# Restream/reindexer

Hardware: AMD Instinct MI355X
Metric: knn_queries_per_sec (higher is better)
Workload: dtype f32; 1 GPU; brute-force KNN, 10000000 x 768 fp32 per GPU, metric=ip, k=10, batch=1 (BASELINE configs[1]); rows_per_gpu=10000000, total_rows=10000000, dim=768, k=10, batch=1, rccl_ranks=0, arch=gfx950:sramecc+:xnack-

## Files before the change

include/rxgpu.h:

```cpp
#ifndef RXGPU_H
#define RXGPU_H

#include <stddef.h>
#include <stdint.h>

#ifdef __cplusplus
extern "C" {
#endif

#define RXGPU_ABI_VERSION 2

typedef enum rxgpu_status {
	RXGPU_OK = 0,
	RXGPU_ERR_PARAMS = -3,
	RXGPU_ERR_LOGIC = -4,
	RXGPU_ERR_NOMEM = -5,
	RXGPU_ERR_DEVICE = -6,
	RXGPU_ERR_NOTFOUND = -7,
	RXGPU_ERR_OVERFLOW = -8
} rxgpu_status;

typedef enum rxgpu_metric { RXGPU_METRIC_L2 = 0, RXGPU_METRIC_IP = 1, RXGPU_METRIC_COSINE = 2 } rxgpu_metric;

typedef struct rxgpu_index rxgpu_index;
// ... 31 lines not shown
uint64_t rxgpu_index_capacity(const rxgpu_index* h);
uint32_t rxgpu_index_dim(const rxgpu_index* h);
uint32_t rxgpu_index_row_stride(const rxgpu_index* h);
int rxgpu_index_metric(const rxgpu_index* h);
int rxgpu_index_device(const rxgpu_index* h);
uint64_t rxgpu_index_device_bytes(const rxgpu_index* h);


int rxgpu_search_knn(rxgpu_index* h, const float* queries, uint32_t nq, uint32_t kk, float* out_dist, uint32_t* out_row,
					 uint32_t* out_count);

int rxgpu_index_upload_row_ids(rxgpu_index* h, uint64_t first_row, uint64_t n, const int32_t* row_ids);
const void* rxgpu_index_row_ids_device(const rxgpu_index* h);
int rxgpu_search_knn_resident(rxgpu_index* h, const float* query, uint32_t kk, void** d_dist, void** d_row, void** d_count, void** stream,
							  uint32_t* entries);
uint32_t rxgpu_index_resident_contexts(rxgpu_index* h);
int rxgpu_search_knn_device(rxgpu_index* h, const void* d_queries, uint32_t nq, uint32_t kk, void* d_out_dist, void* d_out_row,
							void* d_out_count, void* stream);
int rxgpu_scan_policy(uint64_t rows, uint32_t dim, uint32_t nq, int shadow_available, int stats_finite);
int rxgpu_scan_tier(uint64_t rows, uint32_t dim, uint32_t nq, int shadow_available, int stats_finite);
int rxgpu_scan_i6(uint64_t rows, uint32_t dim, uint32_t nq, int i6_available, int stats_finite);
int rxgpu_index_last_candidates(const rxgpu_index* h, uint32_t* out_count, uint32_t* out_cap);
int rxgpu_index_inspect(rxgpu_index* h, const char* what, void* out, uint64_t cap_bytes, uint64_t* out_bytes);

int rxgpu_search_knn_subset(rxgpu_index* h, const float* queries, uint32_t nq, uint32_t kk, const uint32_t* row_ids, uint64_t n_ids,
							float* out_dist, uint32_t* out_row, uint32_t* out_count);
int rxgpu_search_knn_bitmap(rxgpu_index* h, const float* queries, uint32_t nq, uint32_t kk, const uint32_t* allowed_words,
							uint64_t n_words, float* out_dist, uint32_t* out_row, uint32_t* out_count, uint64_t* out_allowed);
int rxgpu_scan_tier_subset(uint64_t n_ids, uint32_t dim, uint32_t nq, uint32_t kk, int shadow_available, int stats_finite);

int rxgpu_index_set_lists(rxgpu_index* h, uint32_t nlist, const uint64_t* list_off, const uint32_t* list_rows);
int rxgpu_search_knn_lists(rxgpu_index* h, rxgpu_index* coarse, const float* query, uint32_t nprobe, uint32_t kk, float* out_dist,
						   uint32_t* out_row, uint32_t* out_count, uint64_t* out_scanned);
int rxgpu_search_range_lists(rxgpu_index* h, rxgpu_index* coarse, const float* query, uint32_t nprobe, float radius, int inclusive, float* out_dist,
							 uint32_t* out_row, uint64_t cap, uint64_t* out_total, uint64_t* out_scanned);

int rxgpu_ivf_assign(rxgpu_index* h, rxgpu_index* coarse, const uint32_t* row_ids, uint64_t first_row, uint64_t n, uint32_t* out_list);
int rxgpu_ivf_kmeans_step(rxgpu_index* h, rxgpu_index* coarse, const uint32_t* row_ids, uint64_t n, float* out_centroids, float* out_hassign,
						  uint32_t* out_assign);
int rxgpu_ivf_read_train_stats(rxgpu_index* h, uint64_t* rows_assigned, uint64_t* steps, double* kernel_ms, double* sums_ms);

int rxgpu_search_knn_subset_device(rxgpu_index* h, const void* d_queries, uint32_t nq, uint32_t kk, const void* d_row_ids,
								   uint64_t n_ids, void* d_out_dist, void* d_out_row, void* d_out_count, void* stream);
int rxgpu_check_row_list_device(rxgpu_index* h, const void* d_row_ids, uint64_t n_ids, void* stream, int32_t* out_ok);

int rxgpu_search_range_subset(rxgpu_index* h, const float* query, float radius, int inclusive, const uint32_t* row_ids, uint64_t n_ids,
// ... 174 lines not shown
```

reindexer_amd/capi.py:

```python
from __future__ import annotations

import ctypes as C
import os
from pathlib import Path

import numpy as np

PKG = Path(__file__).resolve().parent
LIB_PATH = PKG / "librxgpu.so"

METRIC_L2, METRIC_IP, METRIC_COSINE = 0, 1, 2
METRICS = {"l2": METRIC_L2, "ip": METRIC_IP, "inner_product": METRIC_IP, "cosine": METRIC_COSINE}

RXGPU_OK = 0
RXGPU_ERR_PARAMS = -3
RXGPU_ERR_LOGIC = -4
RXGPU_ERR_NOMEM = -5
RXGPU_ERR_DEVICE = -6
RXGPU_ERR_NOTFOUND = -7
RXGPU_ERR_OVERFLOW = -8

_vp, _u32, _u64, _i, _f = C.c_void_p, C.c_uint32, C.c_uint64, C.c_int, C.c_float
_SIGNATURES = {
    "rxgpu_last_error": (C.c_char_p, []),
# ... 17 lines not shown
    "rxgpu_index_adopt_device_rows": (_i, [_vp, _vp, _u64, _u32, _vp]),
    "rxgpu_index_move_row": (_i, [_vp, _u64, _u64]),
    "rxgpu_index_truncate": (_i, [_vp, _u64]),
    "rxgpu_index_count": (_u64, [_vp]),
    "rxgpu_index_capacity": (_u64, [_vp]),
    "rxgpu_index_dim": (_u32, [_vp]),
    "rxgpu_index_row_stride": (_u32, [_vp]),
    "rxgpu_index_metric": (_i, [_vp]),
    "rxgpu_index_device": (_i, [_vp]),
    "rxgpu_index_device_bytes": (_u64, [_vp]),
    "rxgpu_search_knn": (_i, [_vp, _vp, _u32, _u32, _vp, _vp, _vp]),
    "rxgpu_index_upload_row_ids": (_i, [_vp, _u64, _u64, _vp]),
    "rxgpu_index_row_ids_device": (_vp, [_vp]),
    "rxgpu_search_knn_resident": (_i, [_vp, _vp, _u32, C.POINTER(_vp), C.POINTER(_vp), C.POINTER(_vp), C.POINTER(_vp), C.POINTER(_u32)]),
    "rxgpu_index_resident_contexts": (_u32, [_vp]),
    "rxgpu_search_knn_device": (_i, [_vp, _vp, _u32, _u32, _vp, _vp, _vp, _vp]),
    "rxgpu_scan_policy": (_i, [_u64, _u32, _u32, _i, _i]),
    "rxgpu_scan_tier": (_i, [_u64, _u32, _u32, _i, _i]),
    "rxgpu_scan_i6": (_i, [_u64, _u32, _u32, _i, _i]),
    "rxgpu_scan_tier_subset": (_i, [_u64, _u32, _u32, _u32, _i, _i]),
    "rxgpu_scan_tier_range": (_i, [_u64, _u32, _i, _i, _i]),
    "rxgpu_index_last_candidates": (_i, [_vp, C.POINTER(_u32), C.POINTER(_u32)]),
    "rxgpu_index_inspect": (_i, [_vp, C.c_char_p, _vp, _u64, C.POINTER(_u64)]),
    "rxgpu_search_knn_subset": (_i, [_vp, _vp, _u32, _u32, _vp, _u64, _vp, _vp, _vp]),
    "rxgpu_search_knn_bitmap": (_i, [_vp, _vp, _u32, _u32, _vp, _u64, _vp, _vp, _vp, C.POINTER(_u64)]),
    "rxgpu_index_set_lists": (_i, [_vp, _u32, _vp, _vp]),
    "rxgpu_search_knn_lists": (_i, [_vp, _vp, _vp, _u32, _u32, _vp, _vp, _vp, C.POINTER(_u64)]),
    "rxgpu_search_range_lists": (_i, [_vp, _vp, _vp, _u32, C.c_float, _i, _vp, _vp, _u64, C.POINTER(_u64), C.POINTER(_u64)]),
    "rxgpu_ivf_assign": (_i, [_vp, _vp, _vp, _u64, _u64, _vp]),
    "rxgpu_ivf_kmeans_step": (_i, [_vp, _vp, _vp, _u64, _vp, _vp, _vp]),
    "rxgpu_ivf_read_train_stats": (_i, [_vp, C.POINTER(_u64), C.POINTER(_u64), C.POINTER(C.c_double), C.POINTER(C.c_double)]),
    "rxgpu_search_knn_subset_device": (_i, [_vp, _vp, _u32, _u32, _vp, _u64, _vp, _vp, _vp, _vp]),
    "rxgpu_check_row_list_device": (_i, [_vp, _vp, _u64, _vp, C.POINTER(C.c_int32)]),
    "rxgpu_search_range_subset": (_i, [_vp, _vp, _f, _i, _vp, _u64, _vp, _vp, _u64, C.POINTER(_u64)]),
    "rxgpu_merge_shards_device": (_i, [_vp, _u32, _u32, _u32, _u32, _vp, _vp, _vp, _vp]),
    "rxgpu_search_range": (_i, [_vp, _vp, _f, _i, _vp, _vp, _u64, C.POINTER(_u64)]),
    "rxgpu_distances": (_i, [_vp, _vp, _vp, _u32, _vp]),
    "rxgpu_hnsw_attach_graph": (_i, [_vp, _vp, _vp, _vp, _u64, _vp, _u32, _u32, C.c_int32, _u32, _u64]),
    "rxgpu_hnsw_update_deleted": (_i, [_vp, _vp, _u64]),
    "rxgpu_hnsw_patch_graph": (_i, [_vp, _u32, _vp, _vp, _vp, _vp, _vp, C.c_int32, _u32, _u64]),
    "rxgpu_hnsw_search_knn": (_i, [_vp, _vp, _u32, _u32, _u32, _vp, _vp, _vp]),
    "rxgpu_hnsw_search_knn_posted": (_i, [_vp, _vp, _u32, _u32, _vp, _vp, _vp, C.POINTER(C.c_int32)]),
    "rxgpu_hnsw_server_stats": (_i, [_vp, C.POINTER(_u64), C.POINTER(_u64)]),
    "rxgpu_hnsw_server_times": (_i, [_vp, C.POINTER(_u64), C.POINTER(_u64)]),
    "rxgpu_hnsw_read_stats4": (_i, [_vp, _vp]),
    "rxgpu_hnsw_attach_sq8": (_i, [_vp, _vp, _vp, _u64, _f]),
# ... 104 lines not shown
    if n < 0:
        _check(n)
    return n


def device_arch(device: int = 0) -> str:
    buf = C.create_string_buffer(256)
    _check(lib().rxgpu_device_arch(device, buf, 256))
    return buf.value.decode()


def scan_policy(rows: int, dim: int, nq: int = 1, shadow_available: bool = True, stats_finite: bool = True) -> bool:
    return bool(lib().rxgpu_scan_policy(rows, dim, nq, int(shadow_available), int(stats_finite)))


def scan_tier(rows: int, dim: int, nq: int = 1, shadow_available: bool = True, stats_finite: bool = True) -> int:
    return int(lib().rxgpu_scan_tier(rows, dim, nq, int(shadow_available), int(stats_finite)))


def scan_i6(rows: int, dim: int, nq: int = 1, i6_available: bool = True, stats_finite: bool = True) -> bool:
    return bool(lib().rxgpu_scan_i6(rows, dim, nq, int(i6_available), int(stats_finite)))


def scan_tier_range(rows: int, dim: int, listed: bool = False, shadow_available: bool = True, stats_finite: bool = True) -> int:
    return int(lib().rxgpu_scan_tier_range(rows, dim, int(listed), int(shadow_available), int(stats_finite)))


def scan_tier_subset(n_ids: int, dim: int, nq: int = 1, kk: int = 10, shadow_available: bool = True, stats_finite: bool = True) -> int:
    return int(lib().rxgpu_scan_tier_subset(n_ids, dim, nq, kk, int(shadow_available), int(stats_finite)))


def _f32c(a) -> np.ndarray:
    return np.ascontiguousarray(a, dtype=np.float32)


class VectorIndex:

    def __init__(self, metric: int | str, dim: int, capacity: int = 0, device: int = 0):
        if isinstance(metric, str):
            metric = METRICS[metric.lower()]
        self.metric, self.dim = int(metric), int(dim)
        h = _vp()
        _check(lib().rxgpu_index_create(self.metric, self.dim, capacity, device, C.byref(h)))
        self._h = h
        self._keepalive = None

# ... 483 lines not shown
```

reindexer_amd/csrc/knn_batched.hip:

```cpp
#include "knn_i8_quant.h"
#include "knn_kernels.hip.h"
#include "rxgpu_internal.h"

namespace rxgpu {

typedef float f32x16 __attribute__((ext_vector_type(16)));

constexpr int kGemmThreads = 256;
constexpr int kGemmRows = 128;
constexpr int kGemmKS = 32;
constexpr int kLdsStride = kGemmKS + 1;

template <int kMetric, int MT, int kMode, int QS>
__global__ __launch_bounds__(kGemmThreads * QS) void knn_gemm(GemmParams p) {
	extern __shared__ __attribute__((aligned(16))) float lds[];
	constexpr int kThreads = kGemmThreads * QS;
	constexpr int QB = MT / 32 / QS;
	constexpr int kQTile = MT * kLdsStride;
	constexpr int kXTile = kGemmRows * kLdsStride;
	float* q_s = lds;
	float* x_s = lds + 2 * kQTile;
	float* thr_s = x_s + 2 * kXTile;
	float* aux_s = thr_s + MT;
	constexpr int kQLoads = MT * (kGemmKS / 4) / kThreads;
// ... 230 lines not shown
	}
	for (int off = 32; off; off >>= 1) s += __shfl_xor(s, off);
	if (lane == 0) {
		const float mg = query_margin<kMetric, true>(s, dim, stats);
		q_sq[qi] = s;
		margin[qi] = mg;
		cand_cnt[qi] = (s < __builtin_inff() && mg < __builtin_inff()) ? 0u : cap + 1u;
	}
}

template <int kMetric>
__global__ __launch_bounds__(64) void knn_query_prep_i8(const float* src, uint32_t dim, float* qpad, int8_t* planes, uint32_t ld8, const unsigned int* stats,
															 float* q_sq, float* margin, float2* qinfo, uint32_t* cand_cnt, uint32_t cap,
															 const unsigned int* estats, const unsigned int* bad_flag) {
	const uint32_t qi = blockIdx.x;
	const int lane = threadIdx.x;
	const float* q = src + size_t(qi) * dim;
	float* o = qpad + size_t(qi) * ld8;
	int8_t* ph = planes + size_t(qi) * 2 * ld8;
	int8_t* pl = ph + ld8;
	float s = 0.f, mx = 0.f;
	double s64 = 0.0;
	bool bad = false;
	for (uint32_t i = lane; i < ld8; i += 64) {
		const float v = i < dim ? q[i] : 0.f;
		o[i] = v;
		if (i < dim) {
			s = __builtin_fmaf(v, v, s);
			s64 += double(v) * double(v);
			mx = fmaxf(mx, fabsf(v));
			bad |= !(fabsf(v) < __builtin_inff());
		}
	}
	for (int off = 32; off; off >>= 1) {
		s += __shfl_xor(s, off);
		s64 += __shfl_xor(s64, off);
		mx = fmaxf(mx, __shfl_xor(mx, off));
	}
	const float sq = i8_scale(mx, kI8QueryMax);
	double r64 = 0.0;
	for (uint32_t i = lane; i < ld8; i += 64) {
		const float v = i < dim ? q[i] : 0.f;
		const int t = i8_quantize(v, sq, kI8QueryMax);
		int hh, ll;
		i8_split(t, hh, ll);
		ph[i] = int8_t(hh);
		pl[i] = int8_t(ll);
		const double r = i8_residual(v, sq, t);
		r64 += r * r;
	}
	for (int off = 32; off; off >>= 1) r64 += __shfl_xor(r64, off);
	bad = __ballot(bad) != 0;
	if (lane == 0) {
		const float qn = i8_norm_up(s64), rq = i8_norm_up(r64);
		const float mg = i8_margin<kMetric>(s, dim, qn, rq, __uint_as_float(stats[0]), __uint_as_float(stats[1]), __uint_as_float(estats[0]), __uint_as_float(estats[1]));
		q_sq[qi] = s;
		qinfo[qi] = make_float2(sq, qn);
		const bool ok = !bad && stats[2] == 0 && !(bad_flag && *bad_flag != 0) && s < __builtin_inff() && qn < __builtin_inff() && mg < __builtin_inff();
		margin[qi] = ok ? mg : __builtin_inff();
		cand_cnt[qi] = ok ? 0u : cap + 1u;
	}
}

__global__ __launch_bounds__(256) void knn_sample_threshold(const float* dense, uint64_t ns, uint32_t nq, uint32_t kk, const float* margin,
															 float* thr) {
	__shared__ float s_d[4][kMaxFusedK];
	__shared__ uint32_t s_i[4][kMaxFusedK];
	const int lane = threadIdx.x & 63, wave = threadIdx.x >> 6;
	const uint32_t qi = blockIdx.x;
	WaveTopK top;
	top.init(kk);
	if (qi < nq) {
// ... 161 lines not shown
```

reindexer_amd/csrc/knn_scan.hip:

```cpp
#include <algorithm>
#include <type_traits>

#include "knn_kernels.hip.h"
#include "knn_scan_common.hip.h"
#include "rxgpu_internal.h"

#include <cstdlib>

namespace rxgpu {

typedef unsigned int u32x4 __attribute__((ext_vector_type(4)));

constexpr int kMergeThreads = 512;
constexpr int kMergeWaves = kMergeThreads / kWave;
constexpr int kMergeAhead = 8;

__device__ __forceinline__ void block_merge_and_store(WaveTopK2& top, const ScanParams& p, int lane, int wave) {
	__shared__ float s_d[kScanWaves][kMaxFusedK2];
	__shared__ uint32_t s_i[kScanWaves][kMaxFusedK2];
	s_d[wave][lane] = top.d0;
	s_i[wave][lane] = top.i0;
	s_d[wave][64 + lane] = top.d1;
	s_i[wave][64 + lane] = top.i1;
	__syncthreads();
// ... 576 lines not shown
	uint32_t b = __float_as_uint(d);
	if (b == 0x80000000u) b = 0;
	b ^= (b >> 31) ? 0xFFFFFFFFu : 0x80000000u;
	return (static_cast<unsigned long long>(b) << 32) | row;
}
__device__ __forceinline__ void merge_bitonic(unsigned long long* key, float* val, uint32_t n) {
	for (uint32_t k = 2; k <= n; k <<= 1) {
		for (uint32_t j = k >> 1; j > 0; j >>= 1) {
			for (uint32_t t = threadIdx.x; t < n / 2; t += kMergeThreads) {
				const uint32_t i = ((t & ~(j - 1)) << 1) | (t & (j - 1)), l = i | j;
				const unsigned long long x = key[i], y = key[l];
				if ((x > y) == ((i & k) == 0)) {
					key[i] = y;
					key[l] = x;
					const float vx = val[i];
					val[i] = val[l];
					val[l] = vx;
				}
			}
			__syncthreads();
		}
	}
}
template <typename TK>
__device__ void merge_by_insertion(const float* part_dist, const uint32_t* part_row, size_t base, uint32_t total, uint32_t kk, float* out_dist,
								   uint32_t* out_row, uint32_t* out_count, float* s_d, uint32_t* s_i);

template <typename TK>
__device__ __forceinline__ void merge_lists(const float* part_dist, const uint32_t* part_row, uint32_t nlists, uint32_t kk, float* out_dist, uint32_t* out_row,
											uint32_t* out_count, unsigned long long* s_key, float* s_val, uint32_t* s_np) {
	uint32_t& s_n = *s_np;
	const uint32_t tid = threadIdx.x, total = nlists * kk;
	const size_t base = size_t(blockIdx.x) * total;
	bool serial = nlists < kk || nlists > kMergeHeadsMax;
	if (!serial) {
		uint32_t n1 = 64;
		while (n1 < nlists) n1 <<= 1;
		for (uint32_t l = tid; l < n1; l += kMergeThreads) {
			unsigned long long k = ~0ull;
			if (l < nlists) {
				const uint32_t r = part_row[base + size_t(l) * kk];
				if (r != kInvalidRow) k = merge_pair_key(part_dist[base + size_t(l) * kk], r);
			}
			s_key[l] = k;
			s_val[l] = 0.f;
		}
		if (tid == 0) s_n = 0;
		__syncthreads();
		merge_bitonic(s_key, s_val, n1);
		const unsigned long long bound = s_key[kk - 1];
		__syncthreads();
		for (uint32_t l = tid; l < nlists; l += kMergeThreads) {
			const size_t at = base + size_t(l) * kk;
			for (uint32_t e = 0; e < kk; ++e) {
				const uint32_t r = part_row[at + e];
				if (r == kInvalidRow) break;
				const float d = part_dist[at + e];
				const unsigned long long k = merge_pair_key(d, r);
				if (k > bound) break;
				const uint32_t pos = atomicAdd(&s_n, 1u);
				if (pos < kMergeCandMax) {
					s_key[pos] = k;
					s_val[pos] = d;
				}
			}
		}
		__syncthreads();
		const uint32_t n = s_n;
		serial = n > kMergeCandMax;
		if (!serial) {
			uint32_t n2 = 64;
			while (n2 < n) n2 <<= 1;
			for (uint32_t q = n + tid; q < n2; q += kMergeThreads) {
				s_key[q] = ~0ull;
				s_val[q] = 0.f;
			}
			__syncthreads();
			merge_bitonic(s_key, s_val, n2);
			const uint32_t cnt = n < kk ? n : kk;
			for (uint32_t q = tid; q < kk; q += kMergeThreads) {
				out_dist[size_t(blockIdx.x) * kk + q] = q < cnt ? s_val[q] : __builtin_inff();
				out_row[size_t(blockIdx.x) * kk + q] = q < cnt ? uint32_t(s_key[q]) : kInvalidRow;
			}
			if (tid == 0 && out_count) out_count[blockIdx.x] = cnt;
			return;
		}
		__syncthreads();
	}
	merge_by_insertion<TK>(part_dist, part_row, base, total, kk, out_dist, out_row, out_count, s_val, reinterpret_cast<uint32_t*>(s_key));
}

template <typename TK>
__global__ __launch_bounds__(kMergeThreads) void knn_merge_lists(const float* part_dist, const uint32_t* part_row, uint32_t nlists, uint32_t kk,
																  float* out_dist, uint32_t* out_row, uint32_t* out_count, const uint32_t* gate_cnt,
																  uint32_t gate_cap) {
	__shared__ unsigned long long s_key[kMergeHeadsMax];
	__shared__ float s_val[kMergeHeadsMax];
	__shared__ uint32_t s_n;
	if (gate_cnt && gate_cnt[blockIdx.x] <= gate_cap) return;
	merge_lists<TK>(part_dist, part_row, nlists, kk, out_dist, out_row, out_count, s_key, s_val, &s_n);
}

template <typename TK>
__global__ __launch_bounds__(kMergeThreads) void knn_merge_final(const float* cand_dist, const uint32_t* cand_row, const uint32_t* cand_cnt, uint32_t cap,
																  const float* part_dist, const uint32_t* part_row, uint32_t nlists, uint32_t kk,
																  float* out_dist, uint32_t* out_row, uint32_t* out_count) {
	__shared__ unsigned long long s_key[kMergeHeadsMax];
	__shared__ float s_val[kMergeHeadsMax];
	__shared__ uint32_t s_n;
	const uint32_t cnt = cand_cnt[blockIdx.x];
	if (cnt <= cap) {
		merge_fold(cand_dist, cand_row, size_t(blockIdx.x) * cap, cnt, kk, out_dist, out_row, out_count, s_val, reinterpret_cast<uint32_t*>(s_key));
	} else {
		merge_lists<TK>(part_dist, part_row, nlists, kk, out_dist, out_row, out_count, s_key, s_val, &s_n);
	}
}

__device__ __forceinline__ void merge_store_list(const WaveTopK& t, float* d, uint32_t* i, int lane) {
	d[lane] = t.bd;
	i[lane] = t.bi;
	d[64 + lane] = __builtin_inff();
	i[64 + lane] = kInvalidRow;
}
__device__ __forceinline__ void merge_store_list(const WaveTopK2& t, float* d, uint32_t* i, int lane) {
	d[lane] = t.d0;
	i[lane] = t.i0;
	d[64 + lane] = t.d1;
	i[64 + lane] = t.i1;
}
template <typename TK>
__device__ void merge_by_insertion(const float* part_dist, const uint32_t* part_row, size_t base, uint32_t total, uint32_t kk, float* out_dist,
								   uint32_t* out_row, uint32_t* out_count, float* s_d, uint32_t* s_i) {
	const int lane = threadIdx.x & 63, wave = threadIdx.x >> 6;
	TK top;
	top.init(kk);
	for (uint32_t c0 = wave * kWave; c0 < total; c0 += kMergeThreads * kMergeAhead) {
		float cd[kMergeAhead];
		uint32_t ci[kMergeAhead];
// ... 386 lines not shown
void launch_filter_approx(const float* approx, uint64_t n, const float* top_dist, const uint32_t* top_count, uint32_t kk, const float* margin,
						  uint32_t* cand_row, uint32_t* cand_cnt, uint32_t cap, uint32_t nq, int cus, hipStream_t s, const uint32_t* ids) {
	const uint32_t gx = uint32_t(std::max<uint64_t>(1, std::min<uint64_t>((n + 255) / 256, uint64_t(cus) * 8)));
	hipLaunchKernelGGL(knn_filter_approx, dim3(gx, nq), dim3(256), 0, s, approx, n, top_dist, top_count, kk, margin, cand_row, cand_cnt, cap, ids);
}

void launch_filter_emitted(const EmitEntry* emit, const uint32_t* emit_cnt, const EmitPlan& plan, const float* top_dist, const uint32_t* top_count, uint32_t kk,
						   const float* margin, uint32_t* cand_row, uint32_t* cand_cnt, uint32_t cap, uint32_t nq, int cus, hipStream_t s) {
	const uint32_t gx = uint32_t(std::max<uint64_t>(1, std::min<uint64_t>(plan.nwaves, uint64_t(cus) * 8)));
	hipLaunchKernelGGL(knn_filter_emitted, dim3(gx, nq), dim3(256), 0, s, emit, emit_cnt, plan, top_dist, top_count, kk, margin, cand_row, cand_cnt, cap);
}

void launch_merge(const float* part_dist, const uint32_t* part_row, uint32_t total_per_query, uint32_t kk, uint32_t nq, float* out_dist,
				  uint32_t* out_row, uint32_t* out_count, const uint32_t* gate_cnt, uint32_t gate_cap, hipStream_t s) {
	if (kk > uint32_t(kMaxFusedK)) {
		hipLaunchKernelGGL(knn_merge_wide, dim3(nq), dim3(kMergeThreads), 0, s, part_dist, part_row, total_per_query, kk, out_dist, out_row, out_count);
		return;
	}
	hipLaunchKernelGGL(knn_merge, dim3(nq), dim3(kMergeThreads), 0, s, part_dist, part_row, total_per_query, kk, out_dist, out_row, out_count,
					   gate_cnt, gate_cap);
}

void launch_merge_lists(const float* part_dist, const uint32_t* part_row, uint32_t nlists, uint32_t kk, uint32_t nq, float* out_dist, uint32_t* out_row,
						uint32_t* out_count, hipStream_t s, const uint32_t* gate_cnt, uint32_t gate_cap) {
	if (kk > uint32_t(kMaxFusedK)) {
		hipLaunchKernelGGL((knn_merge_lists<WaveTopK2>), dim3(nq), dim3(kMergeThreads), 0, s, part_dist, part_row, nlists, kk, out_dist, out_row, out_count,
						   gate_cnt, gate_cap);
	} else {
		hipLaunchKernelGGL((knn_merge_lists<WaveTopK>), dim3(nq), dim3(kMergeThreads), 0, s, part_dist, part_row, nlists, kk, out_dist, out_row, out_count,
						   gate_cnt, gate_cap);
	}
}

void launch_merge_final(const float* cand_dist, const uint32_t* cand_row, const uint32_t* cand_cnt, uint32_t cap, const float* part_dist,
						const uint32_t* part_row, uint32_t nlists, uint32_t kk, uint32_t nq, float* out_dist, uint32_t* out_row, uint32_t* out_count,
						hipStream_t s) {
	if (kk > uint32_t(kMaxFusedK)) {
		hipLaunchKernelGGL((knn_merge_final<WaveTopK2>), dim3(nq), dim3(kMergeThreads), 0, s, cand_dist, cand_row, cand_cnt, cap, part_dist, part_row, nlists, kk,
						   out_dist, out_row, out_count);
	} else {
		hipLaunchKernelGGL((knn_merge_final<WaveTopK>), dim3(nq), dim3(kMergeThreads), 0, s, cand_dist, cand_row, cand_cnt, cap, part_dist, part_row, nlists, kk,
						   out_dist, out_row, out_count);
	}
}

void launch_merge_shards(const uint32_t* gathered, uint32_t world, uint32_t nq, uint32_t kk, uint32_t shard_rows, float* out_dist,
						 uint32_t* out_row, uint32_t* out_count, hipStream_t s, const uint32_t* slot_base, bool sorted) {
	hipLaunchKernelGGL(knn_merge_shards, dim3(nq), dim3(64), 0, s, gathered, world, nq, kk, shard_rows, slot_base, out_dist, out_row, out_count, sorted ? 1u : 0u);
}

void launch_pack_lists(const float* dist, const uint32_t* row, const uint32_t* count, uint32_t nq, uint32_t k, uint32_t kk, uint32_t* dst_dist, uint32_t* dst_row,
					   hipStream_t s) {
	const uint32_t total = nq * kk;
	if (!total) return;
	hipLaunchKernelGGL(knn_pack_lists, dim3((total + 255) / 256), dim3(256), 0, s, dist, row, count, nq, k, kk, dst_dist, dst_row);
}

void launch_range(int metric, const float* rows, const float* inv_norms, const float* query, uint64_t n, uint32_t stride, uint32_t dim,
				  float radius, int inclusive, float* out_dist, uint32_t* out_row, uint64_t cap, unsigned long long* counter,
				  uint32_t gridx, hipStream_t s) {
	RangeParams p{rows, inv_norms, query, n, stride, dim, radius, inclusive, out_dist, out_row, cap, counter};
	switch (metric) {
		case kL2: hipLaunchKernelGGL((knn_range<kL2>), dim3(gridx), dim3(kScanThreads), 0, s, p); break;
		case kIP: hipLaunchKernelGGL((knn_range<kIP>), dim3(gridx), dim3(kScanThreads), 0, s, p); break;
		default: hipLaunchKernelGGL((knn_range<kCos>), dim3(gridx), dim3(kScanThreads), 0, s, p); break;
// ... 37 lines not shown
```

reindexer_amd/csrc/rxgpu_capi.hip:

```cpp
#include <algorithm>
#include <cstdio>
#include <cstdlib>
#include <cstring>

#include "../../include/rxgpu.h"
#include "knn_kernels.hip.h"
#include "rxgpu_internal.h"

namespace rxgpu {
static thread_local std::string g_err;
void set_error(const std::string& msg) { g_err = msg; }
}

using rxgpu::set_error;

namespace rxgpu {
std::atomic<int> g_resident_kernels{0};
namespace {
std::mutex g_retired_mtx;
std::vector<std::pair<void*, bool>> g_retired;
size_t g_retired_bytes = 0;
}
void drain_retired() {
	std::vector<std::pair<void*, bool>> take;
// ... 222 lines not shown
int rxgpu_scan_tier_subset(uint64_t n_ids, uint32_t dim, uint32_t nq, uint32_t kk, int shadow_available, int stats_finite) {
	return int(rxgpu::scan_policy_tier_subset(n_ids, dim, nq, kk, shadow_available != 0, stats_finite != 0));
}

int rxgpu_scan_tier_range(uint64_t rows, uint32_t dim, int listed, int shadow_available, int stats_finite) {
	return int(rxgpu::scan_policy_tier_range(rows, dim, listed != 0, shadow_available != 0, stats_finite != 0));
}

int rxgpu_index_last_candidates(const rxgpu_index* h, uint32_t* out_count, uint32_t* out_cap) {
	RX_CHECK(h && out_count && out_cap, RXGPU_ERR_PARAMS, "rxgpu_index_last_candidates: null argument");
	*out_count = h->last_cand_count.load();
	*out_cap = h->last_cand_cap.load();
	return RXGPU_OK;
}

int rxgpu_index_inspect(rxgpu_index* h, const char* what, void* out, uint64_t cap_bytes, uint64_t* out_bytes) {
	RX_CHECK(h && what && out_bytes, RXGPU_ERR_PARAMS, "rxgpu_index_inspect: null argument");
	*out_bytes = 0;
	RX_CHECK(!h->shard_set, RXGPU_ERR_PARAMS, "rxgpu_index_inspect: single-device indexes only (inspect the rxgpu_index_shard handles)");
	DeviceGuard dg(h->device);
	return rxgpu::inspect_index(h, what, out, cap_bytes, out_bytes);
}

int rxgpu_device_count(void) {
	int n = 0;
	if (hipGetDeviceCount(&n) != hipSuccess) {
		set_error("hipGetDeviceCount failed");
		return RXGPU_ERR_DEVICE;
	}
	return n;
}

int rxgpu_device_arch(int device, char* name, size_t cap) {
	hipDeviceProp_t prop;
	RX_HIP(hipGetDeviceProperties(&prop, device));
	std::snprintf(name, cap, "%s", prop.gcnArchName);
	return RXGPU_OK;
}

int rxgpu_index_create(int metric, uint32_t dim, uint64_t capacity, int device, rxgpu_index** out) {
	RX_CHECK(out, RXGPU_ERR_PARAMS, "rxgpu_index_create: out is null");
	RX_CHECK(metric >= 0 && metric <= 2, RXGPU_ERR_PARAMS, "rxgpu_index_create: unknown metric");
	RX_CHECK(dim > 0 && dim <= 65535, RXGPU_ERR_PARAMS, "rxgpu_index_create: dimension must be in [1, 65535]");
	RX_CHECK(capacity < 0xFFFFFFFFull, RXGPU_ERR_PARAMS, "rxgpu_index_create: capacity must fit 32-bit rows");
	int ndev = 0;
	RX_HIP(hipGetDeviceCount(&ndev));
// ... 267 lines not shown
```

reindexer_amd/csrc/rxgpu_internal.h:

```cpp
#pragma once

#include <atomic>
#include <hip/hip_runtime.h>
#include <stdint.h>

#include <map>
#include <thread>
#include <mutex>
#include <string>
#include <vector>
#include "ft_packed_decode.h"
#include "ft_merge_plan.h"

namespace rxgpu {

struct ScanParams;

uint32_t scan_grid_x(uint64_t n, int cus);
void launch_scan(int metric, const ScanParams& p, uint32_t nq, uint32_t gridx, hipStream_t s);
struct ScanBf16Params;
bool scan_bf16_supported(uint32_t ld);
uint32_t scan_bf16_grid_x(uint64_t n, int cus);
void launch_scan_bf16(int metric, const ScanBf16Params& p, uint32_t nq, uint32_t gridx, hipStream_t s);
struct ScanI8Params;
// ... 7 lines not shown
void launch_query_prep_i8(int metric, const float* src, uint32_t nq, uint32_t dim, float* qpad, int8_t* planes, uint32_t ld8, const unsigned int* stats,
						  float* q_sq, float* margin, float2* qinfo, uint32_t* cand_cnt, uint32_t cap, hipStream_t s, const unsigned int* estats = nullptr);
struct ScanI6Params;
uint32_t scan_i6_seed_step(uint64_t n);
uint32_t scan_i6_grid_x(uint64_t n, uint32_t set_step, int cus);
void launch_scan_i6(int metric, const ScanI6Params& p, uint32_t nq, uint32_t gridx, hipStream_t s, const ScanI8Emit* emit, bool keep);
void launch_i6_build(const float* rows, const float* inv_norms, uint64_t first_row, uint64_t n, uint32_t stride, uint32_t dim, uint8_t* codes, float2* side,
					 uint32_t ld6, unsigned int* stats6, int cus, hipStream_t s);
void launch_i6_copy_row(uint8_t* codes, uint32_t ld6, uint64_t from, uint64_t to, hipStream_t s);
void launch_filter_approx(const float* approx, uint64_t n, const float* top_dist, const uint32_t* top_count, uint32_t kk, const float* margin,
						  uint32_t* cand_row, uint32_t* cand_cnt, uint32_t cap, uint32_t nq, int cus, hipStream_t s,
						  const uint32_t* ids = nullptr);
struct EmitEntry;
struct EmitPlan;
void launch_filter_emitted(const EmitEntry* emit, const uint32_t* emit_cnt, const EmitPlan& plan, const float* top_dist, const uint32_t* top_count, uint32_t kk,
						   const float* margin, uint32_t* cand_row, uint32_t* cand_cnt, uint32_t cap, uint32_t nq, int cus,
						   hipStream_t s);
void launch_filter_emitted_wide(const EmitEntry* emit, const uint32_t* emit_cnt, const EmitPlan& plan, const float* top_dist, const uint32_t* top_count,
								uint32_t kk, const float* margin, uint32_t* cand_row, uint32_t* cand_cnt, uint32_t cap, uint32_t nq, int cus,
								hipStream_t s);
void launch_merge(const float* part_dist, const uint32_t* part_row, uint32_t total_per_query, uint32_t kk, uint32_t nq, float* out_dist,
				  uint32_t* out_row, uint32_t* out_count, const uint32_t* gate_cnt, uint32_t gate_cap, hipStream_t s);
void launch_merge_lists(const float* part_dist, const uint32_t* part_row, uint32_t nlists, uint32_t kk, uint32_t nq, float* out_dist, uint32_t* out_row,
						uint32_t* out_count, hipStream_t s, const uint32_t* gate_cnt = nullptr,
						uint32_t gate_cap = 0);
void launch_merge_final(const float* cand_dist, const uint32_t* cand_row, const uint32_t* cand_cnt, uint32_t cap, const float* part_dist,
						const uint32_t* part_row, uint32_t nlists, uint32_t kk, uint32_t nq, float* out_dist, uint32_t* out_row, uint32_t* out_count,
						hipStream_t s);
void launch_merge_shards(const uint32_t* gathered, uint32_t world, uint32_t nq, uint32_t kk, uint32_t shard_rows, float* out_dist,
						 uint32_t* out_row, uint32_t* out_count, hipStream_t s, const uint32_t* slot_base = nullptr, bool sorted = true);
void launch_pack_lists(const float* dist, const uint32_t* row, const uint32_t* count, uint32_t nq, uint32_t k, uint32_t kk, uint32_t* dst_dist, uint32_t* dst_row,
					   hipStream_t s);
void launch_range(int metric, const float* rows, const float* inv_norms, const float* query, uint64_t n, uint32_t stride, uint32_t dim,
				  float radius, int inclusive, float* out_dist, uint32_t* out_row, uint64_t cap, unsigned long long* counter,
				  uint32_t gridx, hipStream_t s);
void launch_range_subset(int metric, const float* rows, const float* inv_norms, const float* query, const uint32_t* ids, uint64_t n_ids,
						 uint32_t stride, uint32_t dim, float radius, int inclusive, float* out_dist, uint32_t* out_row, uint64_t cap,
						 unsigned long long* counter, uint32_t gridx, hipStream_t s);
void launch_distances(int metric, const float* rows, const float* inv_norms, const float* query, uint32_t stride, uint32_t dim,
					  const uint32_t* ids, uint32_t n, float* out, hipStream_t s);
struct RangeI8Cand;
void launch_range_i8(int metric, const ScanI8Params& p, const RangeI8Cand& c, const uint32_t* ids, int cus, hipStream_t s);
void launch_range_rescore(int metric, const float* rows, const float* inv_norms, const float* query, const uint32_t* cand_cnt, const uint32_t* cand_row,
						  uint32_t ccap, uint32_t stride, uint32_t dim, float radius, int inclusive, float* out_dist, uint32_t* out_row, uint64_t cap,
						  unsigned long long* counter, uint32_t gridx, hipStream_t s);

uint32_t subset_grid_x(uint64_t n_ids, uint32_t dim, uint32_t kk, int cus);
void launch_scan_subset(int metric, const ScanParams& p, const uint32_t* ids, uint32_t nq, uint32_t gridx, int cus, hipStream_t s);
uint32_t bitmap_tiles(uint64_t n_rows);
void launch_bitmap_count(const uint32_t* words, uint64_t n_rows, uint32_t* tile_scratch, unsigned long long* total, hipStream_t s);
void launch_bitmap_expand(const uint32_t* words, uint64_t n_rows, const uint32_t* tile_scratch, uint32_t* out_rows, uint64_t cap, hipStream_t s);
// ... 548 lines not shown
```

Baseline: 993.1 queries/s.

## Speed up top-k merge with wave-sort heads, rank selection and batched list walks

The merge-lists path now builds its head bound with per-wave register bitonic sorts and a rank-based k-th selection, replacing a full shared-memory bitonic sort. Candidate lists are walked several entries ahead per iteration. The final candidate merge gains a select path that computes a bound from per-wave minima, filters candidates, and writes results by rank, falling back to the old fold on NaN or overflow. Query quantisation prep keeps values in registers instead of reading the query twice, and a probe API reports which merge path ran, at the cost of extra code and more branches.

```diff
diff --git a/include/rxgpu.h b/include/rxgpu.h
--- a/include/rxgpu.h
+++ b/include/rxgpu.h
@@ -77,6 +77,8 @@
 int rxgpu_scan_i6(uint64_t rows, uint32_t dim, uint32_t nq, int i6_available, int stats_finite);
 int rxgpu_index_last_candidates(const rxgpu_index* h, uint32_t* out_count, uint32_t* out_cap);
 int rxgpu_index_inspect(rxgpu_index* h, const char* what, void* out, uint64_t cap_bytes, uint64_t* out_bytes);
+int rxgpu_knn_merge_probe(int device, int what, const float* dist, const uint32_t* row, uint32_t n, uint32_t kk, float* out_dist, uint32_t* out_row,
+						  uint32_t* out_count, int* out_path);
 
 int rxgpu_search_knn_subset(rxgpu_index* h, const float* queries, uint32_t nq, uint32_t kk, const uint32_t* row_ids, uint64_t n_ids,
 							float* out_dist, uint32_t* out_row, uint32_t* out_count);
diff --git a/reindexer_amd/capi.py b/reindexer_amd/capi.py
--- a/reindexer_amd/capi.py
+++ b/reindexer_amd/capi.py
@@ -63,6 +63,7 @@
     "rxgpu_scan_tier_range": (_i, [_u64, _u32, _i, _i, _i]),
     "rxgpu_index_last_candidates": (_i, [_vp, C.POINTER(_u32), C.POINTER(_u32)]),
     "rxgpu_index_inspect": (_i, [_vp, C.c_char_p, _vp, _u64, C.POINTER(_u64)]),
+    "rxgpu_knn_merge_probe": (_i, [_i, _i, _vp, _vp, _u32, _u32, _vp, _vp, C.POINTER(_u32), C.POINTER(_i)]),
     "rxgpu_search_knn_subset": (_i, [_vp, _vp, _u32, _u32, _vp, _u64, _vp, _vp, _vp]),
     "rxgpu_search_knn_bitmap": (_i, [_vp, _vp, _u32, _u32, _vp, _u64, _vp, _vp, _vp, C.POINTER(_u64)]),
     "rxgpu_index_set_lists": (_i, [_vp, _u32, _vp, _vp]),
@@ -213,6 +214,22 @@
     return bool(lib().rxgpu_scan_i6(rows, dim, nq, int(i6_available), int(stats_finite)))
 
 
+MERGE_LISTS, MERGE_CANDIDATES, MERGE_FOLD = 0, 1, 2
+
+
+def knn_merge_probe(what: int, dist: np.ndarray, row: np.ndarray, kk: int, device: int = 0):
+    dist = np.ascontiguousarray(dist, np.float32)
+    row = np.ascontiguousarray(row, np.uint32)
+    assert dist.shape == row.shape
+    n = dist.shape[0] if what == MERGE_LISTS else dist.size
+    assert what != MERGE_LISTS or dist.shape == (n, kk)
+    out_d, out_r = np.empty(kk, np.float32), np.empty(kk, np.uint32)
+    cnt, path = _u32(0), _i(0)
+    _check(lib().rxgpu_knn_merge_probe(device, what, dist.ctypes.data, row.ctypes.data, n, kk, out_d.ctypes.data, out_r.ctypes.data, C.byref(cnt),
+                                       C.byref(path)))
+    return out_d, out_r, int(cnt.value), bool(path.value)
+
+
 def scan_tier_range(rows: int, dim: int, listed: bool = False, shadow_available: bool = True, stats_finite: bool = True) -> int:
     return int(lib().rxgpu_scan_tier_range(rows, dim, int(listed), int(shadow_available), int(stats_finite)))
 
diff --git a/reindexer_amd/csrc/knn_batched.hip b/reindexer_amd/csrc/knn_batched.hip
--- a/reindexer_amd/csrc/knn_batched.hip
+++ b/reindexer_amd/csrc/knn_batched.hip
@@ -276,8 +276,7 @@
 	float s = 0.f, mx = 0.f;
 	double s64 = 0.0;
 	bool bad = false;
-	for (uint32_t i = lane; i < ld8; i += 64) {
-		const float v = i < dim ? q[i] : 0.f;
+	auto measure = [&](uint32_t i, float v) {
 		o[i] = v;
 		if (i < dim) {
 			s = __builtin_fmaf(v, v, s);
@@ -285,16 +284,10 @@
 			mx = fmaxf(mx, fabsf(v));
 			bad |= !(fabsf(v) < __builtin_inff());
 		}
-	}
-	for (int off = 32; off; off >>= 1) {
-		s += __shfl_xor(s, off);
-		s64 += __shfl_xor(s64, off);
-		mx = fmaxf(mx, __shfl_xor(mx, off));
-	}
-	const float sq = i8_scale(mx, kI8QueryMax);
+	};
+	float sq = 0.f;
 	double r64 = 0.0;
-	for (uint32_t i = lane; i < ld8; i += 64) {
-		const float v = i < dim ? q[i] : 0.f;
+	auto quantise = [&](uint32_t i, float v) {
 		const int t = i8_quantize(v, sq, kI8QueryMax);
 		int hh, ll;
 		i8_split(t, hh, ll);
@@ -302,6 +295,38 @@
 		pl[i] = int8_t(ll);
 		const double r = i8_residual(v, sq, t);
 		r64 += r * r;
+	};
+	auto fold = [&] {
+		for (int off = 32; off; off >>= 1) {
+			s += __shfl_xor(s, off);
+			s64 += __shfl_xor(s64, off);
+			mx = fmaxf(mx, __shfl_xor(mx, off));
+		}
+		sq = i8_scale(mx, kI8QueryMax);
+	};
+	constexpr uint32_t kPrepRegs = 16;
+	if (ld8 <= kPrepRegs * 64) {
+		float v[kPrepRegs];
+#pragma unroll
+		for (uint32_t u = 0; u < kPrepRegs; ++u) {
+			const uint32_t i = u * 64 + lane;
+			v[u] = i < dim ? q[i] : 0.f;
+		}
+#pragma unroll
+		for (uint32_t u = 0; u < kPrepRegs; ++u) {
+			const uint32_t i = u * 64 + lane;
+			if (i < ld8) measure(i, v[u]);
+		}
+		fold();
+#pragma unroll
+		for (uint32_t u = 0; u < kPrepRegs; ++u) {
+			const uint32_t i = u * 64 + lane;
+			if (i < ld8) quantise(i, v[u]);
+		}
+	} else {
+		for (uint32_t i = lane; i < ld8; i += 64) measure(i, i < dim ? q[i] : 0.f);
+		fold();
+		for (uint32_t i = lane; i < ld8; i += 64) quantise(i, i < dim ? q[i] : 0.f);
 	}
 	for (int off = 32; off; off >>= 1) r64 += __shfl_xor(r64, off);
 	bad = __ballot(bad) != 0;
diff --git a/reindexer_amd/csrc/knn_scan.hip b/reindexer_amd/csrc/knn_scan.hip
--- a/reindexer_amd/csrc/knn_scan.hip
+++ b/reindexer_amd/csrc/knn_scan.hip
@@ -622,46 +622,138 @@
 		}
 	}
 }
+constexpr uint32_t kMergeRankMax = 256;
+__device__ __forceinline__ unsigned long long merge_wave_sort(unsigned long long k, int lane) {
+	for (int size = 2; size <= kWave; size <<= 1) {
+		for (int j = size >> 1; j > 0; j >>= 1) {
+			const unsigned long long o = __shfl_xor(k, j);
+			const bool take_min = ((lane & size) == 0) == ((lane & j) == 0);
+			k = (k < o) == take_min ? k : o;
+		}
+	}
+	return k;
+}
+__device__ __forceinline__ uint32_t merge_rank(const unsigned long long* key, uint32_t n, uint32_t i) {
+	const unsigned long long mine = key[i];
+	uint32_t rank = 0;
+	for (uint32_t j = 0; j < n; ++j) {
+		const unsigned long long k = key[j];
+		rank += (k < mine || (k == mine && j < i)) ? 1u : 0u;
+	}
+	return rank;
+}
+__device__ __forceinline__ void merge_kth_key(const unsigned long long* key, uint32_t m, uint32_t kk, unsigned long long* bound) {
+	__syncthreads();
+	if (threadIdx.x < m && merge_rank(key, m, threadIdx.x) == kk - 1) *bound = key[threadIdx.x];
+	__syncthreads();
+}
+__device__ __forceinline__ void merge_write_sorted(unsigned long long* s_key, float* s_val, uint32_t n, uint32_t kk, float* out_dist, uint32_t* out_row,
+												   uint32_t* out_count) {
+	const uint32_t tid = threadIdx.x, cnt = n < kk ? n : kk;
+	const size_t o = size_t(blockIdx.x) * kk;
+	if (tid == 0 && out_count) out_count[blockIdx.x] = cnt;
+	if (n <= kMergeRankMax) {
+		if (tid < n) {
+			const uint32_t rank = merge_rank(s_key, n, tid);
+			if (rank < kk) {
+				out_dist[o + rank] = s_val[tid];
+				out_row[o + rank] = uint32_t(s_key[tid]);
+			}
+		}
+		for (uint32_t q = cnt + tid; q < kk; q += kMergeThreads) {
+			out_dist[o + q] = __builtin_inff();
+			out_row[o + q] = kInvalidRow;
+		}
+		return;
+	}
+	uint32_t n2 = 64;
+	while (n2 < n) n2 <<= 1;
+	for (uint32_t q = n + tid; q < n2; q += kMergeThreads) {
+		s_key[q] = ~0ull;
+		s_val[q] = 0.f;
+	}
+	__syncthreads();
+	merge_bitonic(s_key, s_val, n2);
+	for (uint32_t q = tid; q < kk; q += kMergeThreads) {
+		out_dist[o + q] = q < cnt ? s_val[q] : __builtin_inff();
+		out_row[o + q] = q < cnt ? uint32_t(s_key[q]) : kInvalidRow;
+	}
+}
+
 template <typename TK>
 __device__ void merge_by_insertion(const float* part_dist, const uint32_t* part_row, size_t base, uint32_t total, uint32_t kk, float* out_dist,
 								   uint32_t* out_row, uint32_t* out_count, float* s_d, uint32_t* s_i);
 
+constexpr uint32_t kMergeWalkAhead = 4;
 template <typename TK>
-__device__ __forceinline__ void merge_lists(const float* part_dist, const uint32_t* part_row, uint32_t nlists, uint32_t kk, float* out_dist, uint32_t* out_row,
+__device__ __forceinline__ bool merge_lists(const float* part_dist, const uint32_t* part_row, uint32_t nlists, uint32_t kk, float* out_dist, uint32_t* out_row,
 											uint32_t* out_count, unsigned long long* s_key, float* s_val, uint32_t* s_np) {
 	uint32_t& s_n = *s_np;
 	const uint32_t tid = threadIdx.x, total = nlists * kk;
+	const int lane = threadIdx.x & 63, wave = threadIdx.x >> 6;
 	const size_t base = size_t(blockIdx.x) * total;
 	bool serial = nlists < kk || nlists > kMergeHeadsMax;
 	if (!serial) {
-		uint32_t n1 = 64;
-		while (n1 < nlists) n1 <<= 1;
-		for (uint32_t l = tid; l < n1; l += kMergeThreads) {
+		auto head = [&](uint32_t l) {
 			unsigned long long k = ~0ull;
 			if (l < nlists) {
 				const uint32_t r = part_row[base + size_t(l) * kk];
-				if (r != kInvalidRow) k = merge_pair_key(part_dist[base + size_t(l) * kk], r);
-			}
-			s_key[l] = k;
-			s_val[l] = 0.f;
-		}
+				const float d = part_dist[base + size_t(l) * kk];
+				if (r != kInvalidRow) k = merge_pair_key(d, r);
+			}
+			return k;
+		};
+		const uint32_t runs = (nlists + kWave - 1) / kWave, per_run = kk < uint32_t(kWave) ? kk : uint32_t(kWave);
+		unsigned long long bound;
 		if (tid == 0) s_n = 0;
-		__syncthreads();
-		merge_bitonic(s_key, s_val, n1);
-		const unsigned long long bound = s_key[kk - 1];
+		if (nlists <= 2 * kMergeThreads && runs * per_run <= kMergeRankMax) {
+			unsigned long long h0 = head(tid), h1 = head(kMergeThreads + tid);
+			h0 = merge_wave_sort(h0, lane);
+			if (runs > uint32_t(kMergeWaves)) h1 = merge_wave_sort(h1, lane);
+			if (uint32_t(lane) < per_run) {
+				if (uint32_t(wave) < runs) s_key[wave * per_run + lane] = h0;
+				if (uint32_t(kMergeWaves + wave) < runs) s_key[(kMergeWaves + wave) * per_run + lane] = h1;
+			}
+			merge_kth_key(s_key, runs * per_run, kk, &s_key[kMergeRankMax]);
+			bound = s_key[kMergeRankMax];
+		} else {
+			uint32_t n1 = 64;
+			while (n1 < nlists) n1 <<= 1;
+			for (uint32_t l = tid; l < n1; l += kMergeThreads) {
+				s_key[l] = head(l);
+				s_val[l] = 0.f;
+			}
+			__syncthreads();
+			merge_bitonic(s_key, s_val, n1);
+			bound = s_key[kk - 1];
+		}
 		__syncthreads();
 		for (uint32_t l = tid; l < nlists; l += kMergeThreads) {
 			const size_t at = base + size_t(l) * kk;
-			for (uint32_t e = 0; e < kk; ++e) {
-				const uint32_t r = part_row[at + e];
-				if (r == kInvalidRow) break;
-				const float d = part_dist[at + e];
-				const unsigned long long k = merge_pair_key(d, r);
-				if (k > bound) break;
-				const uint32_t pos = atomicAdd(&s_n, 1u);
-				if (pos < kMergeCandMax) {
-					s_key[pos] = k;
-					s_val[pos] = d;
+			bool more = true;
+			for (uint32_t e0 = 0; e0 < kk && more; e0 += kMergeWalkAhead) {
+				uint32_t r[kMergeWalkAhead];
+				float d[kMergeWalkAhead];
+#pragma unroll
+				for (uint32_t u = 0; u < kMergeWalkAhead; ++u) {
+					r[u] = kInvalidRow;
+					d[u] = __builtin_inff();
+					if (e0 + u < kk) {
+						r[u] = part_row[at + e0 + u];
+						d[u] = part_dist[at + e0 + u];
+					}
+				}
+#pragma unroll
+				for (uint32_t u = 0; u < kMergeWalkAhead; ++u) {
+					const unsigned long long k = merge_pair_key(d[u], r[u]);
+					more = more && r[u] != kInvalidRow && k <= bound;
+					if (more) {
+						const uint32_t pos = atomicAdd(&s_n, 1u);
+						if (pos < kMergeCandMax) {
+							s_key[pos] = k;
+							s_val[pos] = d[u];
+						}
+					}
 				}
 			}
 		}
@@ -669,51 +761,125 @@
 		const uint32_t n = s_n;
 		serial = n > kMergeCandMax;
 		if (!serial) {
-			uint32_t n2 = 64;
-			while (n2 < n) n2 <<= 1;
-			for (uint32_t q = n + tid; q < n2; q += kMergeThreads) {
-				s_key[q] = ~0ull;
-				s_val[q] = 0.f;
-			}
-			__syncthreads();
-			merge_bitonic(s_key, s_val, n2);
-			const uint32_t cnt = n < kk ? n : kk;
-			for (uint32_t q = tid; q < kk; q += kMergeThreads) {
-				out_dist[size_t(blockIdx.x) * kk + q] = q < cnt ? s_val[q] : __builtin_inff();
-				out_row[size_t(blockIdx.x) * kk + q] = q < cnt ? uint32_t(s_key[q]) : kInvalidRow;
-			}
-			if (tid == 0 && out_count) out_count[blockIdx.x] = cnt;
-			return;
+			merge_write_sorted(s_key, s_val, n, kk, out_dist, out_row, out_count);
+			return true;
 		}
 		__syncthreads();
 	}
 	merge_by_insertion<TK>(part_dist, part_row, base, total, kk, out_dist, out_row, out_count, s_val, reinterpret_cast<uint32_t*>(s_key));
+	return false;
 }
 
 template <typename TK>
 __global__ __launch_bounds__(kMergeThreads) void knn_merge_lists(const float* part_dist, const uint32_t* part_row, uint32_t nlists, uint32_t kk,
 																  float* out_dist, uint32_t* out_row, uint32_t* out_count, const uint32_t* gate_cnt,
-																  uint32_t gate_cap) {
+																  uint32_t gate_cap, uint32_t* path) {
 	__shared__ unsigned long long s_key[kMergeHeadsMax];
 	__shared__ float s_val[kMergeHeadsMax];
 	__shared__ uint32_t s_n;
 	if (gate_cnt && gate_cnt[blockIdx.x] <= gate_cap) return;
-	merge_lists<TK>(part_dist, part_row, nlists, kk, out_dist, out_row, out_count, s_key, s_val, &s_n);
+	const bool fast = merge_lists<TK>(part_dist, part_row, nlists, kk, out_dist, out_row, out_count, s_key, s_val, &s_n);
+	if (path && threadIdx.x == 0) path[blockIdx.x] = fast ? 1u : 0u;
+}
+
+__device__ __forceinline__ bool merge_select(const float* cand_dist, const uint32_t* cand_row, size_t base, uint32_t cnt, uint32_t kk, float* out_dist,
+											 uint32_t* out_row, uint32_t* out_count, unsigned long long* s_key, float* s_val, uint32_t* s_np) {
+	uint32_t& s_n = *s_np;
+	const uint32_t tid = threadIdx.x;
+	const int lane = threadIdx.x & 63, wave = threadIdx.x >> 6;
+	auto walk = [&](auto&& each) {
+		for (uint32_t c0 = tid; c0 < cnt; c0 += kMergeThreads * kMergeAhead) {
+			float cd[kMergeAhead];
+			uint32_t ci[kMergeAhead];
+#pragma unroll
+			for (int u = 0; u < kMergeAhead; ++u) {
+				const uint32_t c = c0 + uint32_t(u) * kMergeThreads;
+				cd[u] = __builtin_inff();
+				ci[u] = kInvalidRow;
+				if (c < cnt) {
+					cd[u] = cand_dist[base + c];
+					ci[u] = cand_row[base + c];
+				}
+			}
+#pragma unroll
+			for (int u = 0; u < kMergeAhead; ++u) {
+				if (ci[u] != kInvalidRow) each(cd[u], ci[u]);
+			}
+		}
+	};
+	uint32_t& s_nan = *reinterpret_cast<uint32_t*>(&s_val[kMergeHeadsMax - 1]);
+	if (tid == 0) {
+		s_n = 0;
+		s_nan = 0;
+	}
+	__syncthreads();
+	unsigned long long bound = ~0ull;
+	bool nan = false;
+	if (cnt > uint32_t(kMergeThreads)) {
+		unsigned long long h = ~0ull;
+		walk([&](float d, uint32_t r) {
+			nan |= d != d;
+			const unsigned long long k = merge_pair_key(d, r);
+			h = k < h ? k : h;
+		});
+		h = merge_wave_sort(h, lane);
+		if (uint32_t(lane) < kk) s_key[uint32_t(wave) * kk + lane] = h;
+		if (nan) s_nan = 1;
+		__syncthreads();
+		if (s_nan) return false;
+		const uint32_t m = uint32_t(kMergeWaves) * kk;
+		if (m <= kMergeRankMax) {
+			merge_kth_key(s_key, m, kk, &s_key[kMergeRankMax]);
+			bound = s_key[kMergeRankMax];
+		} else {
+			if (tid >= m) s_key[tid] = ~0ull;
+			s_val[tid] = 0.f;
+			__syncthreads();
+			merge_bitonic(s_key, s_val, kMergeThreads);
+			bound = s_key[kk - 1];
+		}
+		if (bound == ~0ull) return false;
+		__syncthreads();
+	}
+	walk([&](float d, uint32_t r) {
+		nan |= d != d;
+		const unsigned long long k = merge_pair_key(d, r);
+		if (k <= bound) {
+			const uint32_t pos = atomicAdd(&s_n, 1u);
+			if (pos < kMergeCandMax) {
+				s_key[pos] = k;
+				s_val[pos] = d;
+			}
+		}
+	});
+	if (nan) s_nan = 1;
+	__syncthreads();
+	if (s_nan) return false;
+	const uint32_t n = s_n;
+	if (n > kMergeCandMax) return false;
+	merge_write_sorted(s_key, s_val, n, kk, out_dist, out_row, out_count);
+	return true;
 }
 
 template <typename TK>
 __global__ __launch_bounds__(kMergeThreads) void knn_merge_final(const float* cand_dist, const uint32_t* cand_row, const uint32_t* cand_cnt, uint32_t cap,
 																  const float* part_dist, const uint32_t* part_row, uint32_t nlists, uint32_t kk,
-																  float* out_dist, uint32_t* out_row, uint32_t* out_count) {
+																  float* out_dist, uint32_t* out_row, uint32_t* out_count, uint32_t* path) {
 	__shared__ unsigned long long s_key[kMergeHeadsMax];
 	__shared__ float s_val[kMergeHeadsMax];
 	__shared__ uint32_t s_n;
 	const uint32_t cnt = cand_cnt[blockIdx.x];
+	bool fast;
 	if (cnt <= cap) {
-		merge_fold(cand_dist, cand_row, size_t(blockIdx.x) * cap, cnt, kk, out_dist, out_row, out_count, s_val, reinterpret_cast<uint32_t*>(s_key));
+		fast = merge_select(cand_dist, cand_row, size_t(blockIdx.x) * cap, cnt, kk, out_dist, out_row, out_count, s_key, s_val, &s_n);
+		if (!fast) {
+			__syncthreads();
+			merge_fold(cand_dist, cand_row, size_t(blockIdx.x) * cap, cnt, kk, out_dist, out_row, out_count, s_val, reinterpret_cast<uint32_t*>(s_key));
+		}
 	} else {
-		merge_lists<TK>(part_dist, part_row, nlists, kk, out_dist, out_row, out_count, s_key, s_val, &s_n);
-	}
+		fast = merge_lists<TK>(part_dist, part_row, nlists, kk, out_dist, out_row, out_count, s_key, s_val, &s_n);
+	}
+	if (path && threadIdx.x == 0) path[blockIdx.x] = fast ? 1u : 0u;
 }
 
 __device__ __forceinline__ void merge_store_list(const WaveTopK& t, float* d, uint32_t* i, int lane) {
@@ -1146,25 +1312,25 @@
 }
 
 void launch_merge_lists(const float* part_dist, const uint32_t* part_row, uint32_t nlists, uint32_t kk, uint32_t nq, float* out_dist, uint32_t* out_row,
-						uint32_t* out_count, hipStream_t s, const uint32_t* gate_cnt, uint32_t gate_cap) {
+						uint32_t* out_count, hipStream_t s, const uint32_t* gate_cnt, uint32_t gate_cap, uint32_t* path) {
 	if (kk > uint32_t(kMaxFusedK)) {
 		hipLaunchKernelGGL((knn_merge_lists<WaveTopK2>), dim3(nq), dim3(kMergeThreads), 0, s, part_dist, part_row, nlists, kk, out_dist, out_row, out_count,
-						   gate_cnt, gate_cap);
+						   gate_cnt, gate_cap, path);
 	} else {
 		hipLaunchKernelGGL((knn_merge_lists<WaveTopK>), dim3(nq), dim3(kMergeThreads), 0, s, part_dist, part_row, nlists, kk, out_dist, out_row, out_count,
-						   gate_cnt, gate_cap);
+						   gate_cnt, gate_cap, path);
 	}
 }
 
 void launch_merge_final(const float* cand_dist, const uint32_t* cand_row, const uint32_t* cand_cnt, uint32_t cap, const float* part_dist,
 						const uint32_t* part_row, uint32_t nlists, uint32_t kk, uint32_t nq, float* out_dist, uint32_t* out_row, uint32_t* out_count,
-						hipStream_t s) {
+						hipStream_t s, uint32_t* path) {
 	if (kk > uint32_t(kMaxFusedK)) {
 		hipLaunchKernelGGL((knn_merge_final<WaveTopK2>), dim3(nq), dim3(kMergeThreads), 0, s, cand_dist, cand_row, cand_cnt, cap, part_dist, part_row, nlists, kk,
-						   out_dist, out_row, out_count);
+						   out_dist, out_row, out_count, path);
 	} else {
 		hipLaunchKernelGGL((knn_merge_final<WaveTopK>), dim3(nq), dim3(kMergeThreads), 0, s, cand_dist, cand_row, cand_cnt, cap, part_dist, part_row, nlists, kk,
-						   out_dist, out_row, out_count);
+						   out_dist, out_row, out_count, path);
 	}
 }
 
diff --git a/reindexer_amd/csrc/rxgpu_capi.hip b/reindexer_amd/csrc/rxgpu_capi.hip
--- a/reindexer_amd/csrc/rxgpu_capi.hip
+++ b/reindexer_amd/csrc/rxgpu_capi.hip
@@ -268,6 +268,49 @@
 	return rxgpu::inspect_index(h, what, out, cap_bytes, out_bytes);
 }
 
+int rxgpu_knn_merge_probe(int device, int what, const float* dist, const uint32_t* row, uint32_t n, uint32_t kk, float* out_dist, uint32_t* out_row,
+						  uint32_t* out_count, int* out_path) {
+	RX_CHECK(out_dist && out_row && out_count && out_path && (n == 0 || (dist && row)), RXGPU_ERR_PARAMS, "rxgpu_knn_merge_probe: null argument");
+	RX_CHECK(what >= 0 && what <= 2, RXGPU_ERR_PARAMS, "rxgpu_knn_merge_probe: unknown kernel");
+	RX_CHECK(kk >= 1 && kk <= uint32_t(what == 0 ? rxgpu::kMaxFusedK2 : rxgpu::kMaxFusedK), RXGPU_ERR_PARAMS, "rxgpu_knn_merge_probe: kk out of range");
+	const uint64_t pairs = what == 0 ? uint64_t(n) * kk : n;
+	RX_CHECK(pairs <= (1u << 24), RXGPU_ERR_PARAMS, "rxgpu_knn_merge_probe: too many pairs");
+	DeviceGuard dg(device);
+	RX_CHECK(dg.ok, RXGPU_ERR_DEVICE, "rxgpu_knn_merge_probe: no such device");
+	const size_t in_words = size_t(std::max<uint64_t>(pairs, 1));
+	uint32_t* d = nullptr;
+	RX_HIP(hipMalloc(reinterpret_cast<void**>(&d), (2 * in_words + 2 * kk + 3) * sizeof(uint32_t)));
+	float* d_dist = reinterpret_cast<float*>(d);
+	uint32_t* d_row = d + in_words;
+	float* d_od = reinterpret_cast<float*>(d_row + in_words);
+	uint32_t* d_or = d_row + in_words + kk;
+	uint32_t* d_tail = d_or + kk;
+	const uint32_t tail[3] = {0, 0, n};
+	hipError_t e = hipMemcpy(d_tail, tail, sizeof(tail), hipMemcpyHostToDevice);
+	if (e == hipSuccess && pairs) e = hipMemcpy(d_dist, dist, pairs * sizeof(float), hipMemcpyHostToDevice);
+	if (e == hipSuccess && pairs) e = hipMemcpy(d_row, row, pairs * sizeof(uint32_t), hipMemcpyHostToDevice);
+	if (e == hipSuccess) {
+		if (what == 0) {
+			rxgpu::launch_merge_lists(d_dist, d_row, n, kk, 1, d_od, d_or, d_tail, nullptr, nullptr, 0, d_tail + 1);
+		} else if (what == 1) {
+			rxgpu::launch_merge_final(d_dist, d_row, d_tail + 2, n, nullptr, nullptr, 0, kk, 1, d_od, d_or, d_tail, nullptr, d_tail + 1);
+		} else {
+			rxgpu::launch_merge(d_dist, d_row, n, kk, 1, d_od, d_or, d_tail, nullptr, 0, nullptr);
+		}
+		e = hipGetLastError();
+	}
+	if (e == hipSuccess) e = hipDeviceSynchronize();
+	uint32_t back[2] = {0, 0};
+	if (e == hipSuccess) e = hipMemcpy(out_dist, d_od, kk * sizeof(float), hipMemcpyDeviceToHost);
+	if (e == hipSuccess) e = hipMemcpy(out_row, d_or, kk * sizeof(uint32_t), hipMemcpyDeviceToHost);
+	if (e == hipSuccess) e = hipMemcpy(back, d_tail, sizeof(back), hipMemcpyDeviceToHost);
+	(void)hipFree(d);
+	RX_HIP(e);
+	*out_count = back[0];
+	*out_path = int(back[1]);
+	return RXGPU_OK;
+}
+
 int rxgpu_device_count(void) {
 	int n = 0;
 	if (hipGetDeviceCount(&n) != hipSuccess) {
diff --git a/reindexer_amd/csrc/rxgpu_internal.h b/reindexer_amd/csrc/rxgpu_internal.h
--- a/reindexer_amd/csrc/rxgpu_internal.h
+++ b/reindexer_amd/csrc/rxgpu_internal.h
@@ -53,11 +53,11 @@
 void launch_merge(const float* part_dist, const uint32_t* part_row, uint32_t total_per_query, uint32_t kk, uint32_t nq, float* out_dist,
 				  uint32_t* out_row, uint32_t* out_count, const uint32_t* gate_cnt, uint32_t gate_cap, hipStream_t s);
 void launch_merge_lists(const float* part_dist, const uint32_t* part_row, uint32_t nlists, uint32_t kk, uint32_t nq, float* out_dist, uint32_t* out_row,
-						uint32_t* out_count, hipStream_t s, const uint32_t* gate_cnt = nullptr,
-						uint32_t gate_cap = 0);
+						uint32_t* out_count, hipStream_t s, const uint32_t* gate_cnt = nullptr, uint32_t gate_cap = 0,
+						uint32_t* path = nullptr);
 void launch_merge_final(const float* cand_dist, const uint32_t* cand_row, const uint32_t* cand_cnt, uint32_t cap, const float* part_dist,
 						const uint32_t* part_row, uint32_t nlists, uint32_t kk, uint32_t nq, float* out_dist, uint32_t* out_row, uint32_t* out_count,
-						hipStream_t s);
+						hipStream_t s, uint32_t* path = nullptr);
 void launch_merge_shards(const uint32_t* gathered, uint32_t world, uint32_t nq, uint32_t kk, uint32_t shard_rows, float* out_dist,
 						 uint32_t* out_row, uint32_t* out_count, hipStream_t s, const uint32_t* slot_base = nullptr, bool sorted = true);
 void launch_pack_lists(const float* dist, const uint32_t* row, const uint32_t* count, uint32_t nq, uint32_t k, uint32_t kk, uint32_t* dst_dist, uint32_t* dst_row,
```

New measurement: 1033 queries/s (median of 6 runs). 4.0% higher.
